# ilyakurdyukov/jpeg-quantsmooth

Measured on AMD Instinct MI355X. Metric: 8x8 blocks/s at q=3 niter=3, higher is better.
Workload: dtype f32

## Files before the change

### jpeg-quantsmooth_amd/csrc/qs_kernels.hip

```cpp
#include <hip/hip_runtime.h>
#include <stdint.h>
#include <stdlib.h>
#include "qs_device.h"
#include "qs_devfn.h"



__device__ __forceinline__ void wave_lds_sync() {
  __builtin_amdgcn_fence(__ATOMIC_RELEASE, "wavefront");
  __builtin_amdgcn_wave_barrier();
  __builtin_amdgcn_fence(__ATOMIC_ACQUIRE, "wavefront");
}

__device__ __forceinline__ uint32_t mulc(uint32_t a, int c) {
  return (uint32_t)__mul24((int)a, c);
}

__device__ __forceinline__ uint32_t lshl13_add(uint32_t x, uint32_t b) {
  uint32_t r;
  asm("v_lshl_add_u32 %0, %1, 13, %2" : "=v"(r) : "v"(x), "v"(b));
  return r;
}

__device__ __forceinline__ void idct8(uint32_t (&v)[8], uint32_t bias) {
  uint32_t z1, z2, z3, z4, z5, t0, t1, t2, t3, e0, e1, e2, e3;
  z2 = v[2]; z3 = v[6];
  z1 = mulc(z2 + z3, 4433);
  asm volatile("" : "+v"(z1));
  t2 = z1 - mulc(z3, 15137);
  t3 = z1 + mulc(z2, 6270);
  t0 = lshl13_add(v[0] + v[4], bias);
  t1 = lshl13_add(v[0] - v[4], bias);
  e0 = t0 + t3; e3 = t0 - t3; e1 = t1 + t2; e2 = t1 - t2;
  t0 = v[7]; t1 = v[5]; t2 = v[3]; t3 = v[1];
  z1 = t0 + t3; z2 = t1 + t2; z3 = t0 + t2; z4 = t1 + t3;
  z5 = mulc(z3 + z4, 9633);
  asm volatile("" : "+v"(z5));
  t0 = mulc(t0, 2446);  t1 = mulc(t1, 16819);
  t2 = mulc(t2, 25172); t3 = mulc(t3, 12299);
  z1 = mulc(z1, 7373);  z2 = mulc(z2, 20995);
  z3 = mulc(z3, 16069); z4 = mulc(z4, 3196);
  z3 = z5 - z3; z4 = z5 - z4;
  t0 += z3 - z1; t1 += z4 - z2; t2 += z3 - z2; t3 += z4 - z1;
  v[0] = e0 + t3; v[7] = e0 - t3;
  v[1] = e1 + t2; v[6] = e1 - t2;
  v[2] = e2 + t1; v[5] = e2 - t1;
  v[3] = e3 + t0; v[4] = e3 - t0;
}

__device__ __forceinline__ void idct_pass1(uint32_t (&ws)[64]) {
#pragma unroll
  for (int x = 0; x < 8; ++x) {
    uint32_t col[8];
#pragma unroll
    for (int j = 0; j < 8; ++j) col[j] = ws[j * 8 + x];
    idct8(col, 1024u);
#pragma unroll
    for (int j = 0; j < 8; ++j) ws[j * 8 + x] = (uint32_t)((int32_t)col[j] >> 11);
  }
}

__device__ __forceinline__ void idct_pass2_row(uint32_t (&row)[8], int (&out)[8]) {
  idct8(row, 257u << 17);
#pragma unroll
  for (int j = 0; j < 8; ++j) {
    int z = (int32_t)row[j];
    z = min(max(z, 0), (256 << 18) - 1);
    out[j] = z >> 18;
  }
}

#define QS_PIX_BITS 0x45000000u
__device__ __forceinline__ void idct_pass2_row_f(uint32_t (&row)[8], float (&out)[8]) {
  idct8(row, 257u << 17);
#pragma unroll
  for (int j = 0; j < 8; ++j) {
    int z = (int32_t)row[j];
    z = min(max(z, 0), (256 << 18) - 1);
    out[j] = __builtin_bit_cast(float, __builtin_amdgcn_alignbit(QS_PIX_BITS >> 14, (uint32_t)z, 18));
  }
}
__device__ __forceinline__ float pix_from_byte(uint32_t v, int n) {
  return __builtin_bit_cast(float, QS_PIX_BITS | ((v >> (8 * n)) & 0xffu));
}

__device__ __forceinline__ void
store_pixel_row(uint8_t* __restrict__ org, int pitch, int y, const int (&o)[8], int bx, int by, int wblk, int hblk,
                int rep_top, int rep_bot) {
  uint2 pk;
  pk.x = (uint32_t)o[0] | ((uint32_t)o[1] << 8) | ((uint32_t)o[2] << 16) | ((uint32_t)o[3] << 24);
  pk.y = (uint32_t)o[4] | ((uint32_t)o[5] << 8) | ((uint32_t)o[6] << 16) | ((uint32_t)o[7] << 24);
  uint8_t* rp = org + (size_t)y * pitch;
  *reinterpret_cast<uint2*>(rp) = pk;
  const bool top = (y == 0 && by == 0 && rep_top), bot = (y == 7 && by == hblk - 1 && rep_bot);
  if (bx == 0) {
    rp[-1] = (uint8_t)o[0];
    if (top) rp[-1 - pitch] = (uint8_t)o[0];
    if (bot) rp[-1 + pitch] = (uint8_t)o[0];
  }
  if (bx == wblk - 1) {
    rp[8] = (uint8_t)o[7];
    if (top) rp[8 - pitch] = (uint8_t)o[7];
    if (bot) rp[8 + pitch] = (uint8_t)o[7];
  }
  if (top) *reinterpret_cast<uint2*>(rp - pitch) = pk;
  if (bot) *reinterpret_cast<uint2*>(rp + pitch) = pk;
}

__device__ __forceinline__ void
idct_ws_to_plane(uint32_t (&ws)[64], uint8_t* __restrict__ plane, int wblk, int hblk, int pitch,
                 int rep_top, int rep_bot, int blk) {
  const int by = blk / wblk, bx = blk - by * wblk;
  idct_pass1(ws);
  uint8_t* org = plane + (size_t)(by * 8 + 1) * pitch + QS_APRON_X + bx * 8;
#pragma unroll
  for (int y = 0; y < 8; ++y) {
    uint32_t row[8]; int o[8];
#pragma unroll
    for (int j = 0; j < 8; ++j) row[j] = ws[y * 8 + j];
    idct_pass2_row(row, o);
    store_pixel_row(org, pitch, y, o, bx, by, wblk, hblk, rep_top, rep_bot);
  }
}

__device__ __forceinline__ void
idct_wave_to_plane(const QsConsts* __restrict__ cst, int16_t* __restrict__ coef,
                   uint8_t* __restrict__ plane, int wblk, int hblk, int pitch,
                   int first, int defer, int rep_top, int rep_bot, int* __restrict__ status, int base, uint32_t* lds) {
  const int lane = threadIdx.x & 63;
  const int nblk = wblk * hblk;
  const int nvec = min(64, nblk - base) * 8;
  uint4* gsrc = reinterpret_cast<uint4*>(coef) + (size_t)base * 8;
  uint4 v[8];
#pragma unroll
  for (int j = 0; j < 8; ++j) {
    const int idx = j * 64 + lane;
    v[j] = make_uint4(0, 0, 0, 0);
    if (idx < nvec) v[j] = gsrc[idx];
  }
  if (first) {
    int q[8], bad = 0;
    qs_load_qraw8(cst, lane & 7, q);
#pragma unroll
    for (int j = 0; j < 8; ++j) v[j] = qs_dequant8<true>(v[j], q, bad);
    if (!defer) {
#pragma unroll
      for (int j = 0; j < 8; ++j) {
        const int idx = j * 64 + lane;
        if (idx < nvec) gsrc[idx] = v[j];
      }
    }
    if (bad) atomicOr(status, 1);
  }
  {
    const int m0 = (lane & 7) * 4;
#pragma unroll
    for (int j = 0; j < 8; ++j) {
      uint32_t* dst = lds + m0 * QS_LDS_PITCH + (j * 8 + (lane >> 3));
      dst[0] = v[j].x; dst[QS_LDS_PITCH] = v[j].y; dst[2 * QS_LDS_PITCH] = v[j].z; dst[3 * QS_LDS_PITCH] = v[j].w;
    }
  }
  wave_lds_sync();
  const uint32_t* col = lds + lane;
  uint32_t ws[64];
#pragma unroll
  for (int r = 0; r < 32; ++r) {
    const uint32_t d = col[r * QS_LDS_PITCH];
    ws[r * 2] = (uint32_t)(int32_t)(int16_t)(d & 0xffff);
    ws[r * 2 + 1] = (uint32_t)((int32_t)d >> 16);
  }
  if (base + lane < nblk) idct_ws_to_plane(ws, plane, wblk, hblk, pitch, rep_top, rep_bot, base + lane);
}

__global__ void __launch_bounds__(256)
qs_idct_plane_kernel(const QsConsts* __restrict__ cst, int16_t* __restrict__ coef,
                     uint8_t* __restrict__ plane, int wblk, int hblk, int pitch,
                     int first, int rep_top, int rep_bot, int* __restrict__ status) {
  __shared__ uint32_t lds_all[4][32 * QS_LDS_PITCH];
  const int wave = threadIdx.x >> 6;
  const int base = __builtin_amdgcn_readfirstlane((int)(blockIdx.x * 256 + wave * 64));
  if (base >= wblk * hblk) return;
  idct_wave_to_plane(cst, coef, plane, wblk, hblk, pitch, first & 1, first & 2, rep_top, rep_bot, status, base, lds_all[wave]);
}

__global__ void __launch_bounds__(256)
qs_idct_set_kernel(const QsPlaneSet set, int first) {
  __shared__ uint32_t lds_all[4][32 * QS_LDS_PITCH];
  const int wave = threadIdx.x >> 6;
  const int w = __builtin_amdgcn_readfirstlane((int)(blockIdx.x * 4 + wave));
  if (w >= set.wave0[set.n]) return;
  const int i = qs_set_find(set, w);
  const QsPlaneRef& r = set.ref[i];
  const int base = (w - set.wave0[i]) * 64;
  if (base >= r.wblk * r.hblk) return;
  idct_wave_to_plane(r.cst, r.coef, r.plane, r.wblk, r.hblk, r.pitch, first, r.mode & QS_PLANE_QUANT,
                     r.mode & QS_PLANE_REP_TOP, r.mode & QS_PLANE_REP_BOT, r.status, base, lds_all[wave]);
}



typedef int16_t __attribute__((may_alias)) lds_i16;
__device__ __forceinline__ int lds_coef(const uint32_t* col, int i) {
  const lds_i16* p = reinterpret_cast<const lds_i16*>(col + (i >> 1) * QS_LDS_PITCH) + (i & 1);
  return *p;
}
__device__ __forceinline__ void lds_set_coef(uint32_t* col, int i, int v) {
  lds_i16* p = reinterpret_cast<lds_i16*>(col + (i >> 1) * QS_LDS_PITCH) + (i & 1);
  *p = (lds_i16)v;
}

static_assert(QS_LDS_PITCH * 4 == 260, "the literal offsets below assume a 260-byte row pitch");
#define QS_LDS16_GROUP(BASE, W, N0) \
  asm volatile("ds_read_i16 %0, %16\n\tds_read_i16 %1, %16 offset:2\n\t" \
               "ds_read_i16 %2, %16 offset:260\n\tds_read_i16 %3, %16 offset:262\n\t" \
               "ds_read_i16 %4, %16 offset:520\n\tds_read_i16 %5, %16 offset:522\n\t" \
               "ds_read_i16 %6, %16 offset:780\n\tds_read_i16 %7, %16 offset:782\n\t" \
               "ds_read_i16 %8, %16 offset:1040\n\tds_read_i16 %9, %16 offset:1042\n\t" \
               "ds_read_i16 %10, %16 offset:1300\n\tds_read_i16 %11, %16 offset:1302\n\t" \
               "ds_read_i16 %12, %16 offset:1560\n\tds_read_i16 %13, %16 offset:1562\n\t" \
               "ds_read_i16 %14, %16 offset:1820\n\tds_read_i16 %15, %16 offset:1822\n\t" \
               "s_waitcnt lgkmcnt(0)" \
               : "=&v"(W[(N0) + 0]), "=&v"(W[(N0) + 1]), "=&v"(W[(N0) + 2]), "=&v"(W[(N0) + 3]), \
                 "=&v"(W[(N0) + 4]), "=&v"(W[(N0) + 5]), "=&v"(W[(N0) + 6]), "=&v"(W[(N0) + 7]), \
                 "=&v"(W[(N0) + 8]), "=&v"(W[(N0) + 9]), "=&v"(W[(N0) + 10]), "=&v"(W[(N0) + 11]), \
                 "=&v"(W[(N0) + 12]), "=&v"(W[(N0) + 13]), "=&v"(W[(N0) + 14]), "=&v"(W[(N0) + 15]) \
               : "v"(BASE) : "memory")
__device__ __forceinline__ void lds_read_block_i16(const uint32_t* col, uint32_t (&ws)[64]) {
  typedef const __attribute__((address_space(3))) uint32_t* lds_ptr;
  const uint32_t a0 = (uint32_t)(uintptr_t)(lds_ptr)col;
  const uint32_t a1 = a0 + 8 * 260, a2 = a0 + 16 * 260, a3 = a0 + 24 * 260;
  QS_LDS16_GROUP(a0, ws, 0);
  QS_LDS16_GROUP(a1, ws, 16);
  QS_LDS16_GROUP(a2, ws, 32);
  QS_LDS16_GROUP(a3, ws, 48);
}

#define QS_PIX_SCALE 0.000244140625f
#define QS_TERM_D(D, W) { \
    float u_ = __builtin_amdgcn_fmed3f(Rs - __builtin_fabsf(D), 0.0f, 1.0f); \
    float t_ = u_ * u_; \
    float x_ = (D) * t_; \
    float y_ = (W) * t_; \
    num = num + x_ * y_; \
    den = den + y_ * y_; }
#define QS_TERM(A, B, W) { float d_ = (A) - (B); QS_TERM_D(d_, W) }

typedef float qs_w16 __attribute__((ext_vector_type(16)));
typedef int qs_i4 __attribute__((ext_vector_type(4)));
#define QS_SWAIT(BUF) asm volatile("s_waitcnt lgkmcnt(0)" : "+s"(BUF) : : "memory")

#define QS_WAVES_PER_WG 4
#define QS_SMOOTH_MIN_WAVES 3
#define QS_RESIDENT_WG (256 * QS_SMOOTH_MIN_WAVES * 4 / QS_WAVES_PER_WG)
#define QS_PRIO_SLOW 3
#define QS_PRIO_TERMS 0

#define QS_TERM_OPT(COND, A, B, W) { float d_, t_; \
        asm volatile( \
          "s_cmp_lg_u32 %[c], 0\n\t" \
          "s_cbranch_scc1 1f\n\t" \
          "v_sub_f32 %[d], %[a], %[b]\n\t" \
          "v_sub_f32 %[t], %[r], |%[d]| clamp\n\t" \
          "v_mul_f32 %[t], %[t], %[t]\n\t" \
          "v_mul_f32 %[d], %[d], %[t]\n\t" \
          "v_mul_f32 %[t], %[w], %[t]\n\t" \
          "v_mul_f32 %[d], %[d], %[t]\n\t" \
          "v_add_f32 %[n], %[n], %[d]\n\t" \
          "v_mul_f32 %[d], %[t], %[t]\n\t" \
          "v_add_f32 %[e], %[e], %[d]\n" \
          "1:" \
          : [n] "+v"(num), [e] "+v"(den), [d] "=&v"(d_), [t] "=&v"(t_) \
          : [a] "v"(A), [b] "v"(B), [w] "s"(W), [r] "s"(Rs), [c] "s"(COND) : "scc"); }
#define QS_TERM_ASM(A, B, W) { float d_, t_; \
        asm volatile( \
          "v_sub_f32 %[d], %[a], %[b]\n\t" \
          "v_sub_f32 %[t], %[r], |%[d]| clamp\n\t" \
          "v_mul_f32 %[t], %[t], %[t]\n\t" \
          "v_mul_f32 %[d], %[d], %[t]\n\t" \
          "v_mul_f32 %[t], %[w], %[t]\n\t" \
          "v_mul_f32 %[d], %[d], %[t]\n\t" \
          "v_add_f32 %[n], %[n], %[d]\n\t" \
          "v_mul_f32 %[d], %[t], %[t]\n\t" \
          "v_add_f32 %[e], %[e], %[d]" \
          : [n] "+v"(num), [e] "+v"(den), [d] "=&v"(d_), [t] "=&v"(t_) \
          : [a] "v"(A), [b] "v"(B), [w] "s"(W), [r] "s"(Rs)); }

#define QS_TERM_D_ASM(D, W) { float d_, t_; \
        asm volatile( \
          "v_sub_f32 %[t], %[r], |%[a]| clamp\n\t" \
          "v_mul_f32 %[t], %[t], %[t]\n\t" \
          "v_mul_f32 %[d], %[a], %[t]\n\t" \
          "v_mul_f32 %[t], %[w], %[t]\n\t" \
          "v_mul_f32 %[d], %[d], %[t]\n\t" \
          "v_add_f32 %[n], %[n], %[d]\n\t" \
          "v_mul_f32 %[d], %[t], %[t]\n\t" \
          "v_add_f32 %[e], %[e], %[d]" \
          : [n] "+v"(num), [e] "+v"(den), [d] "=&v"(d_), [t] "=&v"(t_) \
          : [a] "v"(D), [w] "s"(W), [r] "s"(Rs)); }
#define QS_HOIST 20
#ifndef QS_HOIST_DIAG
#define QS_HOIST_DIAG 32
#endif
#ifndef QS_Q1_SKIP
#define QS_Q1_SKIP 1
#endif
#ifndef QS_STASH
#define QS_STASH 1
#endif

#define QS_SMOOTH_KERNEL_NAME qs_smooth_plane_kernel
#include "qs_smooth_kernel.inc"
#undef QS_SMOOTH_KERNEL_NAME
#define QS_SMOOTH_KERNEL_NAME qs_smooth_set_kernel
#define QS_SMOOTH_SET 1
#include "qs_smooth_kernel.inc"
#undef QS_SMOOTH_KERNEL_NAME
#undef QS_SMOOTH_SET

#define QS_DP_KERNEL_NAME qs_smooth_dp_kernel
#include "qs_smooth_dp_kernel.inc"
#undef QS_DP_KERNEL_NAME
#define QS_DP_KERNEL_NAME qs_smooth_dp_set_kernel
#define QS_DP_SET 1
#include "qs_smooth_dp_kernel.inc"
#undef QS_DP_KERNEL_NAME
#undef QS_DP_SET

__global__ void __launch_bounds__(256)
qs_clamp_kernel(int16_t* __restrict__ coef, size_t nvec) {
  size_t i = (size_t)blockIdx.x * 256 + threadIdx.x;
  const size_t stride = (size_t)gridDim.x * 256;
  uint4* p = reinterpret_cast<uint4*>(coef);
  for (; i < nvec; i += stride) {
    uint4 v = p[i];
    uint32_t d[4] = {v.x, v.y, v.z, v.w};
#pragma unroll
    for (int c = 0; c < 4; ++c) {
      int lo = (int16_t)(d[c] & 0xffff), hi = (int32_t)d[c] >> 16;
      lo = min(max(lo, -1023), 1023); hi = min(max(hi, -1023), 1023);
      d[c] = ((uint32_t)lo & 0xffffu) | ((uint32_t)hi << 16);
    }
    p[i] = make_uint4(d[0], d[1], d[2], d[3]);
  }
}

__global__ void __launch_bounds__(256)
qs_dequant_kernel(const QsConsts* __restrict__ cst, int16_t* __restrict__ coef, size_t nvec) {
  size_t i = (size_t)blockIdx.x * 256 + threadIdx.x;
  const size_t stride = (size_t)gridDim.x * 256;
  uint4* p = reinterpret_cast<uint4*>(coef);
  for (; i < nvec; i += stride) {
    uint4 v = p[i];
    uint32_t d[4] = {v.x, v.y, v.z, v.w};
    const int j = (int)(i & 7);
#pragma unroll
    for (int c = 0; c < 4; ++c) {
      int lo = (int16_t)(d[c] & 0xffff), hi = (int32_t)d[c] >> 16;
      lo *= cst->qraw[j * 8 + c * 2]; hi *= cst->qraw[j * 8 + c * 2 + 1];
      d[c] = ((uint32_t)lo & 0xffffu) | ((uint32_t)hi << 16);
    }
    p[i] = make_uint4(d[0], d[1], d[2], d[3]);
  }
}

#include "qs_launch.h"

void qs_launch_idct_plane(const QsConsts* cst, int16_t* coef, uint8_t* plane, int wblk, int hblk,
                          int first, int rep_top, int rep_bot, int* status, hipStream_t s) {
  const int nblk = wblk * hblk;
  const int f = first == 3 ? 3 : first ? 1 : 0;
  hipLaunchKernelGGL(qs_idct_plane_kernel, dim3((nblk + 255) / 256), dim3(256), 0, s,
                     cst, coef, plane, wblk, hblk, qs_plane_pitch(wblk), f, rep_top, rep_bot, status);
}

#define QS_DP_WAVES 4
static int qs_dp_waves(int groups) {
  static const int on = [] { const char* v = getenv("QS_HIP_DP"); return v ? atoi(v) : 1; }();
  static const int lim = [] { const char* v = getenv("QS_HIP_DP_GROUPS"); return v ? atoi(v) : 768; }();
  static const int lim2 = [] { const char* v = getenv("QS_HIP_DP_GROUPS2"); return v ? atoi(v) : 1536; }();
  if (!on) return 0;
  return groups <= lim ? QS_DP_WAVES : groups <= lim2 ? 2 : 0;
}

void qs_launch_smooth_plane(const QsConsts* cst, int16_t* coef, const uint8_t* plane, uint8_t* plane_next, int rep_top, int rep_bot,
                            int wblk, int hblk, int diag, int rebalance, int final_clamp, int blk_begin, int blk_end, hipStream_t s) {
  const int n = blk_end - blk_begin;
  if (n <= 0) return;
  const int pitch = qs_plane_pitch(wblk);
  const int rep = (rep_top ? QS_PLANE_REP_TOP : 0) | (rep_bot ? QS_PLANE_REP_BOT : 0);
  if (const int nw = qs_dp_waves((n + 63) / 64)) {
    const dim3 g((n + 63) / 64), b(64 * nw);
#define QS_GO_DP(D, W) hipLaunchKernelGGL((qs_smooth_dp_kernel<D, W>), g, b, 0, s, cst, coef, plane, plane_next, rep, wblk, hblk, pitch, rebalance, final_clamp, blk_begin, blk_end)
    if (nw == 2) { if (diag) QS_GO_DP(true, 2); else QS_GO_DP(false, 2); }
    else if (diag) QS_GO_DP(true, QS_DP_WAVES); else QS_GO_DP(false, QS_DP_WAVES);
#undef QS_GO_DP
    return;
  }
  const int per_wg = 64 * QS_WAVES_PER_WG;
  const dim3 grid((n + per_wg - 1) / per_wg), block(per_wg);
#define QS_GO(K) hipLaunchKernelGGL(K, grid, block, 0, s, cst, coef, plane, plane_next, rep, wblk, hblk, pitch, rebalance, final_clamp, blk_begin, blk_end)
  if (diag) QS_GO(qs_smooth_plane_kernel<true>); else QS_GO(qs_smooth_plane_kernel<false>);
#undef QS_GO
}

void qs_launch_idct_set(const QsPlaneSet& set, int first, hipStream_t s) {
  const int nw = set.wave0[set.n];
  if (nw <= 0) return;
  hipLaunchKernelGGL(qs_idct_set_kernel, dim3((nw + 3) / 4), dim3(256), 0, s, set, first);
}

void qs_launch_smooth_set(const QsPlaneSet& set, int diag, int final_clamp, hipStream_t s) {
  const int nw = set.wave0[set.n];
  if (nw <= 0) return;
  if (const int dw = qs_dp_waves(nw)) {
    const dim3 g(nw), b(64 * dw);
#define QS_GO_DP(D, W) hipLaunchKernelGGL((qs_smooth_dp_set_kernel<D, W>), g, b, 0, s, set, final_clamp)
    if (dw == 2) { if (diag) QS_GO_DP(true, 2); else QS_GO_DP(false, 2); }
    else if (diag) QS_GO_DP(true, QS_DP_WAVES); else QS_GO_DP(false, QS_DP_WAVES);
#undef QS_GO_DP
    return;
  }
  const dim3 grid((nw + QS_WAVES_PER_WG - 1) / QS_WAVES_PER_WG), block(64 * QS_WAVES_PER_WG);
  if (diag) hipLaunchKernelGGL(qs_smooth_set_kernel<true>, grid, block, 0, s, set, final_clamp);
  else      hipLaunchKernelGGL(qs_smooth_set_kernel<false>, grid, block, 0, s, set, final_clamp);
}

void qs_launch_clamp(int16_t* coef, size_t nblk, hipStream_t s) {
  const size_t nvec = nblk * 8;
  const int grid = (int)((nvec + 255) / 256 < 8192 ? (nvec + 255) / 256 : 8192);
  hipLaunchKernelGGL(qs_clamp_kernel, dim3(grid ? grid : 1), dim3(256), 0, s, coef, nvec);
}

void qs_launch_dequant(const QsConsts* cst, int16_t* coef, size_t nblk, hipStream_t s) {
  const size_t nvec = nblk * 8;
  const int grid = (int)((nvec + 255) / 256 < 8192 ? (nvec + 255) / 256 : 8192);
  hipLaunchKernelGGL(qs_dequant_kernel, dim3(grid ? grid : 1), dim3(256), 0, s, cst, coef, nvec);
}
```

### jpeg-quantsmooth_amd/csrc/qs_smooth_kernel.inc

```
template <bool DIAG>
__global__ void __launch_bounds__(64 * QS_WAVES_PER_WG, QS_SMOOTH_MIN_WAVES)
#ifdef QS_SMOOTH_SET
QS_SMOOTH_KERNEL_NAME(const QsPlaneSet set, int final_clamp) {
  __shared__ uint32_t lds_all[QS_WAVES_PER_WG][32 * QS_LDS_PITCH];
#if QS_STASH
  __shared__ uint32_t stash_all[QS_WAVES_PER_WG][2 * 8 * 64];
#endif
  const int lane = threadIdx.x & 63, wave = threadIdx.x >> 6;
  uint32_t* lds = lds_all[wave];
  uint32_t* col = lds + lane;
  const int gw = __builtin_amdgcn_readfirstlane((int)(blockIdx.x * QS_WAVES_PER_WG + wave));
  if (gw >= set.wave0[set.n]) return;
  const int pi = qs_set_find(set, gw);
  const QsConsts* __restrict__ cst = set.ref[pi].cst;
  int16_t* __restrict__ coef = set.ref[pi].coef;
  const uint8_t* __restrict__ plane = set.ref[pi].plane;
  const int wblk = set.ref[pi].wblk, hblk = set.ref[pi].hblk, pitch = set.ref[pi].pitch;
  const int rebalance = set.ref[pi].mode & QS_PLANE_REBALANCE;
  const int nblk = wblk * hblk;
  const int base = (gw - set.wave0[pi]) * 64;
  (void)hblk;
#else
QS_SMOOTH_KERNEL_NAME(const QsConsts* __restrict__ cst, int16_t* __restrict__ coef,
                       const uint8_t* __restrict__ plane, uint8_t* __restrict__ plane_next, int rep,
                       int wblk, int hblk, int pitch,
                       int rebalance, int final_clamp, int blk_begin, int blk_end) {
  __shared__ uint32_t lds_all[QS_WAVES_PER_WG][32 * QS_LDS_PITCH];
#if QS_STASH
  __shared__ uint32_t stash_all[QS_WAVES_PER_WG][2 * 8 * 64];
#endif
  const int lane = threadIdx.x & 63, wave = threadIdx.x >> 6;
  uint32_t* lds = lds_all[wave];
  uint32_t* col = lds + lane;
  const int nblk = blk_end;
  const int base = blk_begin + (blockIdx.x * QS_WAVES_PER_WG + wave) * 64;
#endif
  if (base >= nblk) return;
  const int tail_prio = __builtin_amdgcn_readfirstlane(
      (gridDim.x > QS_RESIDENT_WG && blockIdx.x >= (gridDim.x / QS_RESIDENT_WG) * QS_RESIDENT_WG) ? 1 : 0);
  const int nvec = min(64, nblk - base) * 8;
#ifdef QS_STAGGER
  { unsigned hwid; asm volatile("s_getreg_b32 %0, hwreg(HW_REG_HW_ID)" : "=s"(hwid)); if (hwid & 1u) __builtin_amdgcn_s_sleep(QS_STAGGER); }
#endif

  uint4* gsrc = reinterpret_cast<uint4*>(coef) + (size_t)base * 8;
#ifdef QS_SMOOTH_SET
  if (set.ref[pi].mode & QS_PLANE_QUANT) {
    const int m0 = (lane & 7) * 4;
    int q[8], unused = 0;
    qs_load_qraw8(cst, lane & 7, q);
#pragma unroll
    for (int j = 0; j < 8; ++j) {
      const int idx = j * 64 + lane;
      uint4 v = make_uint4(0, 0, 0, 0);
      if (idx < nvec) v = gsrc[idx];
      v = qs_dequant8<false>(v, q, unused);
      uint32_t* dst = lds + m0 * QS_LDS_PITCH + (j * 8 + (lane >> 3));
      dst[0] = v.x; dst[QS_LDS_PITCH] = v.y; dst[2 * QS_LDS_PITCH] = v.z; dst[3 * QS_LDS_PITCH] = v.w;
    }
  } else
#endif
  {
    const int m0 = (lane & 7) * 4;
#pragma unroll
    for (int j = 0; j < 8; ++j) {
      const int idx = j * 64 + lane;
      uint4 v = make_uint4(0, 0, 0, 0);
      if (idx < nvec) v = gsrc[idx];
      uint32_t* dst = lds + m0 * QS_LDS_PITCH + (j * 8 + (lane >> 3));
      dst[0] = v.x; dst[QS_LDS_PITCH] = v.y; dst[2 * QS_LDS_PITCH] = v.z; dst[3 * QS_LDS_PITCH] = v.w;
    }
  }

  const int blk = min(base + lane, nblk - 1);
  const int by = blk / wblk, bx = blk - by * wblk;
  const uint8_t* org = plane + (size_t)(by * 8 + 1) * pitch + QS_APRON_X + bx * 8;
  uint32_t edge[8];
  {
    const uint2 t = *reinterpret_cast<const uint2*>(org - pitch);
    const uint2 b = *reinterpret_cast<const uint2*>(org + (size_t)8 * pitch);
    edge[0] = t.x; edge[1] = t.y; edge[2] = b.x; edge[3] = b.y;
    uint32_t l[8], r[8];
#pragma unroll
    for (int y = 0; y < 8; ++y) {
      l[y] = org[(ptrdiff_t)y * pitch - 1];
      r[y] = org[(ptrdiff_t)y * pitch + 8];
    }
    edge[4] = l[0] | (l[1] << 8) | (l[2] << 16) | (l[3] << 24);
    edge[5] = l[4] | (l[5] << 8) | (l[6] << 16) | (l[7] << 24);
    edge[6] = r[0] | (r[1] << 8) | (r[2] << 16) | (r[3] << 24);
    edge[7] = r[4] | (r[5] << 8) | (r[6] << 16) | (r[7] << 24);
  }
  wave_lds_sync();

  constexpr int TS = DIAG ? 272 : 160;
  float px[64];
  float bd[32];
  constexpr int NH = DIAG ? QS_HOIST_DIAG : QS_HOIST;
  float hd[NH];

  int kfirst = 63;
#if QS_STASH
  int stash_hi = 0;
#endif
  uint32_t chg = 0;
  long long reb_m0 = 0, reb_m1 = 0;
  const float* tabp = cst->tab;
  const int32_t* recp = &cst->rec[0][0];
  qs_w16 WA, WB;
  qs_i4 REC;
  qs_i4 RECN;
  asm volatile("s_load_dwordx4 %0, %2, %3\n\ts_load_dwordx16 %1, %4, %5\n\ts_waitcnt lgkmcnt(0)"
               : "=&s"(REC), "=&s"(WA) : "s"(recp), "s"(63u * 16u), "s"(tabp), "s"((uint32_t)63 * (TS * 4)) : "memory");
  RECN = REC;

#pragma unroll 1
  for (int g = 0; g < 14; ++g) {
    __builtin_amdgcn_s_setprio(QS_PRIO_SLOW);
    if (g == 0 || __builtin_amdgcn_ballot_w64(chg != 0) != 0) {
      chg = 0;
      uint32_t ws[64];
      lds_read_block_i16(col, ws);
#if QS_STASH
      {
        uint32_t* stash = stash_all[wave] + lane;
#pragma unroll
        for (int x = 0; x < 8; ++x) {
          uint32_t c[8];
          const bool low = x <= 1, high = x >= 6;
          const int slot = (x == 0 || x == 7) ? 0 : 1;
          bool reuse = false, store = false;
          if (low) { reuse = g >= 1 && g <= 7 - x; store = g == 0; }
          if (high) {
            const int fin = 15 - x;
            const bool have = (stash_hi >> (x - 6)) & 1;
            reuse = g >= fin && have; store = g >= fin && !have;
          }
          if ((low || high) && reuse) {
#pragma unroll
            for (int j = 0; j < 8; ++j) c[j] = stash[(slot * 8 + j) * 64];
          } else {
#pragma unroll
            for (int j = 0; j < 8; ++j) c[j] = ws[j * 8 + x];
            idct8(c, 1024u);
#pragma unroll
            for (int j = 0; j < 8; ++j) c[j] = (uint32_t)((int32_t)c[j] >> 11);
            if ((low || high) && store) {
#pragma unroll
              for (int j = 0; j < 8; ++j) stash[(slot * 8 + j) * 64] = c[j];
              if (high) stash_hi |= 1 << (x - 6);
            }
          }
#pragma unroll
          for (int j = 0; j < 8; ++j) ws[j * 8 + x] = c[j];
        }
      }
#else
      idct_pass1(ws);
#endif
#pragma unroll
      for (int y = 0; y < 8; ++y) {
        uint32_t row[8]; float o[8];
#pragma unroll
        for (int j = 0; j < 8; ++j) row[j] = ws[y * 8 + j];
        idct_pass2_row_f(row, o);
#pragma unroll
        for (int j = 0; j < 8; ++j) px[y * 8 + j] = o[j];
      }
#pragma unroll
      for (int e = 0; e < 8; ++e) asm volatile("" : "+v"(edge[e]));
#pragma unroll
      for (int x = 0; x < 8; ++x) {
        bd[x]      = px[x]         - pix_from_byte(edge[0 + (x >> 2)], x & 3);
        bd[8 + x]  = px[56 + x]    - pix_from_byte(edge[2 + (x >> 2)], x & 3);
        bd[16 + x] = px[x * 8]     - pix_from_byte(edge[4 + (x >> 2)], x & 3);
        bd[24 + x] = px[x * 8 + 7] - pix_from_byte(edge[6 + (x >> 2)], x & 3);
      }
#pragma unroll
      for (int t = 0; t < NH; ++t) hd[t] = px[(t / 7) * 8 + t % 7] - px[(t / 7) * 8 + t % 7 + 1];
    }
    const int len = min(g + 1, 15 - g);
    const int klast = max(kfirst - len + 1, 1);
#pragma unroll 1
    for (int k = kfirst; k >= klast; --k) {
#pragma unroll
      for (int p = 0; p < 64; ++p) asm volatile("" : "+v"(px[p]));
      const int md = REC[3];
      const int x2k = (REC[0] >> 16) & 31, qk = REC[1] & 0xffff, x1k = REC[1] >> 16;
      const uint32_t lds_off = ((uint32_t)md >> QS_REC_LDS_SHIFT) & 0x3fffu;
      int rs_bits = REC[2];
      asm volatile("" : "+s"(rs_bits));
      const float Rs = __builtin_bit_cast(float, rs_bits);
      const uint32_t kb = (uint32_t)k * (TS * 4);
      const uint32_t kb_nxt = kb - (uint32_t)(TS * 4);
      const uint32_t kb_s = (uint32_t)__builtin_amdgcn_readfirstlane((int)kb);
      const uint32_t kb_nxt_s = (uint32_t)__builtin_amdgcn_readfirstlane((int)kb_nxt);
      const uint32_t next_first = kb_nxt + (((uint32_t)md >> QS_REC_NXT_SHIFT) & 0x100u);
      const uint32_t after_V = DIAG ? kb + 640u : next_first;
      const uint32_t after_B = (md & QS_REC_V_ANY) ? kb + 384u : after_V;
#if QS_Q1_SKIP
      if (__builtin_expect(md & QS_REC_Q1, 0)) {
        {
          const int c0 = *reinterpret_cast<lds_i16*>(reinterpret_cast<char*>(col) + lds_off);
          reb_m0 += (long long)(c0 * c0);
          reb_m1 += (long long)(c0 * c0);
        }
        asm volatile("s_load_dwordx16 %0, %2, %3\n\ts_load_dwordx4 %1, %4, %5\n\ts_waitcnt lgkmcnt(0)"
                     : "=&s"(WA), "=&s"(RECN)
                     : "s"(tabp), "s"((uint32_t)__builtin_amdgcn_readfirstlane((int)next_first)), "s"(recp),
                       "s"((uint32_t)(k - 1) * 16u) : "memory");
        REC = RECN;
      } else
#endif
      {
      float num = 0.0f, den = 0.0f;
      asm volatile("s_setprio %c1\n\ts_cmp_eq_u32 %0, 0\n\ts_cbranch_scc1 1f\n\ts_setprio %c2\n1:"
                   : : "s"(tail_prio), "i"(QS_PRIO_TERMS), "i"(QS_PRIO_TERMS + 1) : "scc");

#define QS_ROW_D(W, Y) { \
        _Pragma("unroll") for (int x = 0; x < 7; ++x) { \
          QS_TERM(px[(Y) * 8 + x], px[(Y) * 8 + x + 9], W[x]) \
          QS_TERM(px[(Y) * 8 + x + 1], px[(Y) * 8 + x + 8], W[8 + x]) } }
#define QS_EDGE16(W, J0) { \
        _Pragma("unroll") for (int j = 0; j < 16; ++j) QS_TERM_D(bd[(J0) + j], W[j]) }
#define QS_HOISTED_TERM(T, WT) else if ((T) < NH) QS_TERM_D_ASM(hd[(T) % NH], WT)
#define QS_ROWS_H_M(W, Y0, MODE) { \
        _Pragma("unroll") for (int yy = 0; yy < 2; ++yy) \
        _Pragma("unroll") for (int x = 0; x < 7; ++x) { \
          if (((MODE) == 2 && (x & 1)) || ((MODE) == 1 && x == 3)) {} \
          QS_HOISTED_TERM(((Y0) + yy) * 7 + x, W[yy * 8 + x]) \
          else QS_TERM_ASM(px[((Y0) + yy) * 8 + x], px[((Y0) + yy) * 8 + x + 1], W[yy * 8 + x]) } }
#define QS_ROWS_V_M(W, Y0, NY, MODE) { \
        _Pragma("unroll") for (int yy = 0; yy < (NY); ++yy) \
        _Pragma("unroll") for (int x = 0; x < 8; ++x) { \
          if (((MODE) == 2 && (((Y0) + yy) & 1)) || ((MODE) == 1 && (Y0) + yy == 3)) {} \
          else QS_TERM_ASM(px[((Y0) + yy) * 8 + x], px[((Y0) + yy) * 8 + x + 8], W[yy * 8 + x]) } }

      const uint32_t rec_next = (uint32_t)(k - 1) * 16u;
#define QS_ISSUE(NXT, BYTEOFF) \
      asm volatile("s_load_dwordx16 %0, %3, %4" : "=&s"(NXT), "+v"(num), "+v"(den) \
                   : "s"(tabp), "s"((uint32_t)__builtin_amdgcn_readfirstlane((int)(BYTEOFF))) : "memory")
#define QS_ISSUE_K(NXT, IMM) \
      asm volatile("s_load_dwordx16 %0, %3, %4 offset:%c5" : "=&s"(NXT), "+v"(num), "+v"(den) \
                   : "s"(tabp), "s"(kb_s), "i"(IMM) : "memory")
#define QS_LAND(NXT) asm volatile("s_waitcnt lgkmcnt(0)" : "+s"(NXT), "+v"(num), "+v"(den) : : "memory")
#define QS_ISSUE_R(NXT, BYTEOFF) \
      asm volatile("s_load_dwordx16 %0, %4, %5\n\ts_load_dwordx4 %1, %6, %7" : "=&s"(NXT), "=&s"(RECN), "+v"(num), "+v"(den) \
                   : "s"(tabp), "s"((uint32_t)__builtin_amdgcn_readfirstlane((int)(BYTEOFF))), "s"(recp), "s"(rec_next) : "memory")
#define QS_LAND_R(NXT) asm volatile("s_waitcnt lgkmcnt(0)" : "+s"(NXT), "+s"(RECN), "+v"(num), "+v"(den) : : "memory")
#define QS_T4(O) "s_load_dword %1, %4, %5 offset:" #O "\n\ts_load_dword %1, %4, %5 offset:" #O "+0x40\n\ts_load_dword %1, %4, %5 offset:" #O "+0x80\n\ts_load_dword %1, %4, %5 offset:" #O "+0xc0\n\t"
#define QS_ISSUE_T(NXT, IMM) \
      uint32_t touch; \
      if (DIAG) asm volatile("s_load_dwordx16 %0, %4, %6 offset:%c7\n\t" QS_T4(0x0) QS_T4(0x100) QS_T4(0x200) QS_T4(0x300) "s_load_dword %1, %4, %5 offset:0x400" \
                   : "=&s"(NXT), "=&s"(touch), "+v"(num), "+v"(den) \
                   : "s"(tabp), "s"(kb_nxt_s), "s"(kb_s), "i"(IMM) : "memory"); \
      else      asm volatile("s_load_dwordx16 %0, %4, %6 offset:%c7\n\t" QS_T4(0x0) QS_T4(0x100) "s_load_dword %1, %4, %5 offset:0x200\n\ts_load_dword %1, %4, %5 offset:0x240" \
                   : "=&s"(NXT), "=&s"(touch), "+v"(num), "+v"(den) \
                   : "s"(tabp), "s"(kb_nxt_s), "s"(kb_s), "i"(IMM) : "memory")
#define QS_LAND_T(NXT) asm volatile("s_waitcnt lgkmcnt(0)" : "+s"(NXT), "+s"(touch), "+v"(num), "+v"(den) : : "memory")
#define QS_H_SECTION(MODE) { \
        QS_ISSUE_K(WB, 64);  QS_ROWS_H_M(WA, 0, MODE) QS_LAND(WB); \
        QS_ISSUE_K(WA, 128); QS_ROWS_H_M(WB, 2, MODE) QS_LAND(WA); \
        QS_ISSUE_K(WB, 192); QS_ROWS_H_M(WA, 4, MODE) QS_LAND(WB); \
        QS_ISSUE_K(WA, 256); QS_ROWS_H_M(WB, 6, MODE) QS_LAND(WA); }
      if (md & QS_REC_H_ANY) {
        if (md & QS_REC_H_SKIP4) QS_H_SECTION(2)
        else if (md & QS_REC_H_EVEN) QS_H_SECTION(1)
        else QS_H_SECTION(0)
      }
      QS_ISSUE_T(WB, 320); QS_EDGE16(WA, 0) QS_LAND_T(WB);
      if (!DIAG && !(md & QS_REC_V_ANY)) { QS_ISSUE_R(WA, after_B); QS_EDGE16(WB, 16) QS_LAND_R(WA); }
      else                   { QS_ISSUE(WA, after_B);   QS_EDGE16(WB, 16) QS_LAND(WA); }
#define QS_V_SECTION(MODE) { \
        QS_ISSUE_K(WB, 448); QS_ROWS_V_M(WA, 0, 2, MODE) QS_LAND(WB); \
        QS_ISSUE_K(WA, 512); QS_ROWS_V_M(WB, 2, 2, MODE) QS_LAND(WA); \
        QS_ISSUE_K(WB, 576); QS_ROWS_V_M(WA, 4, 2, MODE) QS_LAND(WB); \
        if (!DIAG) { QS_ISSUE_R(WA, after_V); QS_ROWS_V_M(WB, 6, 1, MODE) QS_LAND_R(WA); } \
        else       { QS_ISSUE(WA, after_V);   QS_ROWS_V_M(WB, 6, 1, MODE) QS_LAND(WA); } }
      if (md & QS_REC_V_ANY) {
        if (md & QS_REC_V_SKIP4) QS_V_SECTION(2)
        else if (md & QS_REC_V_EVEN) QS_V_SECTION(1)
        else QS_V_SECTION(0)
      }
      if (DIAG) {
        QS_ISSUE_K(WB, 704);  QS_ROW_D(WA, 0) QS_LAND(WB);
        QS_ISSUE_K(WA, 768);  QS_ROW_D(WB, 1) QS_LAND(WA);
        QS_ISSUE_K(WB, 832);  QS_ROW_D(WA, 2) QS_LAND(WB);
        QS_ISSUE_K(WA, 896);  QS_ROW_D(WB, 3) QS_LAND(WA);
        QS_ISSUE_K(WB, 960);  QS_ROW_D(WA, 4) QS_LAND(WB);
        QS_ISSUE_K(WA, 1024); QS_ROW_D(WB, 5) QS_LAND(WA);
        QS_ISSUE_R(WB, next_first); QS_ROW_D(WA, 6) QS_LAND_R(WB);
        WA = WB;
      }
#undef QS_ROWS_H_M
#undef QS_HOISTED_TERM
#undef QS_ROWS_V_M
#undef QS_H_SECTION
#undef QS_V_SECTION
#undef QS_ISSUE
#undef QS_ISSUE_K
#undef QS_LAND
#undef QS_ISSUE_R
#undef QS_LAND_R
#undef QS_ISSUE_T
#undef QS_LAND_T
#undef QS_T4

      __builtin_amdgcn_s_setprio(QS_PRIO_SLOW);
      lds_i16* const cptr = reinterpret_cast<lds_i16*>(reinterpret_cast<char*>(col) + lds_off);
      const int c0 = *cptr;
      const int r = f2i_x86(round_half_away((num / den) * 4096.0f));
      {
        int orig, lo, hi;
        interval(c0, qk, x1k, x2k, orig, lo, hi);
        int v = (int)((uint32_t)c0 - (uint32_t)r);
        v = min(max(v, lo), hi);
        *cptr = (lds_i16)v;
        chg |= (uint32_t)(v ^ c0);
        if (rebalance) {
          reb_m0 += (long long)(v * orig);
          reb_m1 += (long long)(orig * orig);
        }
      }
      REC = RECN;
      }
    }
    kfirst = klast - 1;
  }
  QS_SWAIT(WA);

  if (rebalance) {
    const long long m0 = reb_m0, m1 = reb_m1;
    if (m1 > m0) {
      const int mul = (int)(((m1 << 13) + (m0 >> 1)) / m0);
#pragma unroll 9
      for (int n = 1; n < 64; ++n) {
        const int c = lds_coef(col, n);
        int orig, lo, hi;
        interval(c, cst->qn[n], cst->x1n[n], cst->x2n[n], orig, lo, hi);
        int v = (c * mul + 0x1000) >> 13;
        v = min(max(v, lo), hi);
        lds_set_coef(col, n, v);
      }
    }
  }
  wave_lds_sync();

  {
    int lane2 = lane;
    asm volatile("" : "+v"(lane2));
    const int lane = lane2;
    const int m0 = (lane & 7) * 4;
#pragma unroll
    for (int j = 0; j < 8; ++j) {
      const int idx = j * 64 + lane;
      const uint32_t* s = lds + m0 * QS_LDS_PITCH + (j * 8 + (lane >> 3));
      uint32_t d[4] = {s[0], s[QS_LDS_PITCH], s[2 * QS_LDS_PITCH], s[3 * QS_LDS_PITCH]};
      if (final_clamp) {
#pragma unroll
        for (int c = 0; c < 4; ++c) {
          int lo = (int16_t)(d[c] & 0xffff), hi = (int32_t)d[c] >> 16;
          lo = min(max(lo, -1023), 1023); hi = min(max(hi, -1023), 1023);
          d[c] = ((uint32_t)lo & 0xffffu) | ((uint32_t)hi << 16);
        }
      }
      if (idx < nvec) gsrc[idx] = make_uint4(d[0], d[1], d[2], d[3]);
    }
  }

#ifdef QS_SMOOTH_SET
  int pi2 = pi;
  asm volatile("" : "+s"(pi2));
  uint8_t* __restrict__ plane_next = set.ref[pi2].plane_next;
  const int rep = set.ref[pi2].mode, wblk2 = set.ref[pi2].wblk, hblk2 = set.ref[pi2].hblk, pitch2 = set.ref[pi2].pitch;
#else
  const int wblk2 = wblk, hblk2 = hblk, pitch2 = pitch;
#endif
  if (plane_next) {
    uint32_t ws[64];
    lds_read_block_i16(col, ws);
    if (base + lane < nblk)
      idct_ws_to_plane(ws, plane_next, wblk2, hblk2, pitch2, rep & QS_PLANE_REP_TOP, rep & QS_PLANE_REP_BOT, base + lane);
  }
}

#undef QS_ROW_D
#undef QS_EDGE16
```

Measured before the change: 276.3 million.

## Precompute pixel differences and move per-lane state to LDS in non-diagonal smoothing

For the non-diagonal kernel variant, the 64-entry pixel array is replaced with precomputed horizontal and vertical difference arrays. The edge bytes, stash and rebalance accumulators move into a per-wave LDS extension, with the accumulators updated through wave-scope LDS atomics, and the change test becomes a wave ballot. The aim is to cut VGPR use and per-term subtraction work so the kernel fits three waves per SIMD. A slow path recomputes the rebalance sums and widens the intervals when large coefficients could overflow, and a Python script is added to check the VGPR, scratch and LDS budget. The extra LDS per wave and the atomic traffic could reduce occupancy or add latency.

```diff
diff --git a/jpeg-quantsmooth_amd/csrc/check_kernel_budget.py b/jpeg-quantsmooth_amd/csrc/check_kernel_budget.py
--- /dev/null
+++ b/jpeg-quantsmooth_amd/csrc/check_kernel_budget.py
@@ -0,0 +1,49 @@
+#!/usr/bin/env python3
+import re
+import sys
+
+KERNELS = ("qs_smooth_plane_kernel", "qs_smooth_set_kernel")
+MAX_VGPRS = 168
+MAX_LDS = 160 * 1024 // 3
+FIELDS = ("group_segment_fixed_size", "private_segment_fixed_size", "vgpr_count")
+
+
+def kernel_records(text):
+    m = re.search(r"^\s*\.amdgpu_metadata\s*$(.*?)^\s*\.end_amdgpu_metadata\s*$", text, re.S | re.M)
+    if not m:
+        return {}
+    recs, cur = [], None
+    for line in m.group(1).split("\n"):
+        if re.match(r"  - \.", line):
+            cur = {}
+            recs.append(cur)
+            line = "    " + line[4:]
+        f = re.match(r"    \.(\w+):\s*(\S+)\s*$", line)
+        if f and cur is not None:
+            cur[f.group(1)] = f.group(2)
+    return {r["name"]: {k: int(r[k]) for k in FIELDS if k in r} for r in recs if "name" in r}
+
+
+def main(path):
+    recs = {n: r for n, r in kernel_records(open(path).read()).items() if any(k in n for k in KERNELS)}
+    if len(recs) != 4 or any(len(r) != len(FIELDS) for r in recs.values()):
+        print(f"check_kernel_budget: ERROR: expected the metadata of 4 recovery kernels in {path}, found {sorted(recs)}", file=sys.stderr)
+        return 1
+    bad = 0
+    for n, r in sorted(recs.items()):
+        why = []
+        if r["private_segment_fixed_size"] != 0:
+            why.append(f"{r['private_segment_fixed_size']} B of scratch per lane (spills)")
+        if r["vgpr_count"] > MAX_VGPRS:
+            why.append(f"{r['vgpr_count']} VGPRs > {MAX_VGPRS} (three waves per SIMD)")
+        if r["group_segment_fixed_size"] > MAX_LDS:
+            why.append(f"{r['group_segment_fixed_size']} B of LDS > {MAX_LDS} (three workgroups per CU)")
+        print(f"check_kernel_budget: {n}: {r['vgpr_count']} VGPRs, {r['private_segment_fixed_size']} B scratch, "
+              f"{r['group_segment_fixed_size']} B LDS" + (" -- ERROR: " + "; ".join(why) if why else ""),
+              file=sys.stderr if why else sys.stdout)
+        bad += bool(why)
+    return 1 if bad else 0
+
+
+if __name__ == "__main__":
+    sys.exit(main(sys.argv[1]))
diff --git a/jpeg-quantsmooth_amd/csrc/qs_kernels.hip b/jpeg-quantsmooth_amd/csrc/qs_kernels.hip
--- a/jpeg-quantsmooth_amd/csrc/qs_kernels.hip
+++ b/jpeg-quantsmooth_amd/csrc/qs_kernels.hip
@@ -210,15 +210,15 @@
 }
 
 static_assert(QS_LDS_PITCH * 4 == 260, "the literal offsets below assume a 260-byte row pitch");
-#define QS_LDS16_GROUP(BASE, W, N0) \
-  asm volatile("ds_read_i16 %0, %16\n\tds_read_i16 %1, %16 offset:2\n\t" \
-               "ds_read_i16 %2, %16 offset:260\n\tds_read_i16 %3, %16 offset:262\n\t" \
-               "ds_read_i16 %4, %16 offset:520\n\tds_read_i16 %5, %16 offset:522\n\t" \
-               "ds_read_i16 %6, %16 offset:780\n\tds_read_i16 %7, %16 offset:782\n\t" \
-               "ds_read_i16 %8, %16 offset:1040\n\tds_read_i16 %9, %16 offset:1042\n\t" \
-               "ds_read_i16 %10, %16 offset:1300\n\tds_read_i16 %11, %16 offset:1302\n\t" \
-               "ds_read_i16 %12, %16 offset:1560\n\tds_read_i16 %13, %16 offset:1562\n\t" \
-               "ds_read_i16 %14, %16 offset:1820\n\tds_read_i16 %15, %16 offset:1822\n\t" \
+#define QS_LDS16_GROUP(BASE, W, N0, O) \
+  asm volatile("ds_read_i16 %0, %16 offset:" #O "\n\tds_read_i16 %1, %16 offset:" #O "+2\n\t" \
+               "ds_read_i16 %2, %16 offset:" #O "+260\n\tds_read_i16 %3, %16 offset:" #O "+262\n\t" \
+               "ds_read_i16 %4, %16 offset:" #O "+520\n\tds_read_i16 %5, %16 offset:" #O "+522\n\t" \
+               "ds_read_i16 %6, %16 offset:" #O "+780\n\tds_read_i16 %7, %16 offset:" #O "+782\n\t" \
+               "ds_read_i16 %8, %16 offset:" #O "+1040\n\tds_read_i16 %9, %16 offset:" #O "+1042\n\t" \
+               "ds_read_i16 %10, %16 offset:" #O "+1300\n\tds_read_i16 %11, %16 offset:" #O "+1302\n\t" \
+               "ds_read_i16 %12, %16 offset:" #O "+1560\n\tds_read_i16 %13, %16 offset:" #O "+1562\n\t" \
+               "ds_read_i16 %14, %16 offset:" #O "+1820\n\tds_read_i16 %15, %16 offset:" #O "+1822\n\t" \
                "s_waitcnt lgkmcnt(0)" \
                : "=&v"(W[(N0) + 0]), "=&v"(W[(N0) + 1]), "=&v"(W[(N0) + 2]), "=&v"(W[(N0) + 3]), \
                  "=&v"(W[(N0) + 4]), "=&v"(W[(N0) + 5]), "=&v"(W[(N0) + 6]), "=&v"(W[(N0) + 7]), \
@@ -229,10 +229,18 @@
   typedef const __attribute__((address_space(3))) uint32_t* lds_ptr;
   const uint32_t a0 = (uint32_t)(uintptr_t)(lds_ptr)col;
   const uint32_t a1 = a0 + 8 * 260, a2 = a0 + 16 * 260, a3 = a0 + 24 * 260;
-  QS_LDS16_GROUP(a0, ws, 0);
-  QS_LDS16_GROUP(a1, ws, 16);
-  QS_LDS16_GROUP(a2, ws, 32);
-  QS_LDS16_GROUP(a3, ws, 48);
+  QS_LDS16_GROUP(a0, ws, 0, 0);
+  QS_LDS16_GROUP(a1, ws, 16, 0);
+  QS_LDS16_GROUP(a2, ws, 32, 0);
+  QS_LDS16_GROUP(a3, ws, 48, 0);
+}
+__device__ __forceinline__ void lds_read_block_i16_1(const uint32_t* col, uint32_t (&ws)[64]) {
+  typedef const __attribute__((address_space(3))) uint32_t* lds_ptr;
+  const uint32_t a0 = (uint32_t)(uintptr_t)(lds_ptr)col;
+  QS_LDS16_GROUP(a0, ws, 0, 0);
+  QS_LDS16_GROUP(a0, ws, 16, 2080);
+  QS_LDS16_GROUP(a0, ws, 32, 4160);
+  QS_LDS16_GROUP(a0, ws, 48, 6240);
 }
 
 #define QS_PIX_SCALE 0.000244140625f
@@ -297,7 +305,6 @@
           "v_add_f32 %[e], %[e], %[d]" \
           : [n] "+v"(num), [e] "+v"(den), [d] "=&v"(d_), [t] "=&v"(t_) \
           : [a] "v"(D), [w] "s"(W), [r] "s"(Rs)); }
-#define QS_HOIST 20
 #ifndef QS_HOIST_DIAG
 #define QS_HOIST_DIAG 32
 #endif
@@ -307,6 +314,22 @@
 #ifndef QS_STASH
 #define QS_STASH 1
 #endif
+#define QS_X_STASH 0
+#define QS_X_EDGE 8
+#define QS_X_REB 16
+#define QS_X_DWORDS 20
+static_assert(QS_WAVES_PER_WG * (32 * QS_LDS_PITCH + QS_X_DWORDS * 64) * 4 <= 160 * 1024 / 3, "LDS budget of three workgroups per CU");
+typedef unsigned long long __attribute__((address_space(3))) qs_lds_u64;
+__device__ __forceinline__ void qs_lds_add64(qs_lds_u64* p, long long v) {
+  __hip_atomic_fetch_add(p, (unsigned long long)v, __ATOMIC_RELAXED, __HIP_MEMORY_SCOPE_WAVEFRONT);
+}
+__device__ __forceinline__ qs_lds_u64* qs_xreb(const uint32_t* col, const uint32_t* lds, int n) {
+  typedef const __attribute__((address_space(3))) uint32_t* lds_ptr;
+  uint32_t a = (uint32_t)(uintptr_t)(lds_ptr)col;
+  asm volatile("" : "+v"(a));
+  const uint32_t b = (uint32_t)(uintptr_t)(lds_ptr)lds;
+  return (qs_lds_u64*)(a * 2u - b + (uint32_t)((32 * QS_LDS_PITCH + (QS_X_REB + 2 * n) * 64) * 4));
+}
 
 #define QS_SMOOTH_KERNEL_NAME qs_smooth_plane_kernel
 #include "qs_smooth_kernel.inc"
diff --git a/jpeg-quantsmooth_amd/csrc/qs_smooth_kernel.inc b/jpeg-quantsmooth_amd/csrc/qs_smooth_kernel.inc
--- a/jpeg-quantsmooth_amd/csrc/qs_smooth_kernel.inc
+++ b/jpeg-quantsmooth_amd/csrc/qs_smooth_kernel.inc
@@ -2,11 +2,11 @@
 __global__ void __launch_bounds__(64 * QS_WAVES_PER_WG, QS_SMOOTH_MIN_WAVES)
 #ifdef QS_SMOOTH_SET
 QS_SMOOTH_KERNEL_NAME(const QsPlaneSet set, int final_clamp) {
-  __shared__ uint32_t lds_all[QS_WAVES_PER_WG][32 * QS_LDS_PITCH];
+  __shared__ __attribute__((aligned(16))) uint32_t lds_all[QS_WAVES_PER_WG][32 * QS_LDS_PITCH + (DIAG ? 0 : QS_X_DWORDS * 64)];
 #if QS_STASH
   __shared__ uint32_t stash_all[QS_WAVES_PER_WG][2 * 8 * 64];
 #endif
-  const int lane = threadIdx.x & 63, wave = threadIdx.x >> 6;
+  const int lane = threadIdx.x & 63, wave = DIAG ? (int)(threadIdx.x >> 6) : __builtin_amdgcn_readfirstlane((int)(threadIdx.x >> 6));
   uint32_t* lds = lds_all[wave];
   uint32_t* col = lds + lane;
   const int gw = __builtin_amdgcn_readfirstlane((int)(blockIdx.x * QS_WAVES_PER_WG + wave));
@@ -25,11 +25,11 @@
                        const uint8_t* __restrict__ plane, uint8_t* __restrict__ plane_next, int rep,
                        int wblk, int hblk, int pitch,
                        int rebalance, int final_clamp, int blk_begin, int blk_end) {
-  __shared__ uint32_t lds_all[QS_WAVES_PER_WG][32 * QS_LDS_PITCH];
+  __shared__ __attribute__((aligned(16))) uint32_t lds_all[QS_WAVES_PER_WG][32 * QS_LDS_PITCH + (DIAG ? 0 : QS_X_DWORDS * 64)];
 #if QS_STASH
   __shared__ uint32_t stash_all[QS_WAVES_PER_WG][2 * 8 * 64];
 #endif
-  const int lane = threadIdx.x & 63, wave = threadIdx.x >> 6;
+  const int lane = threadIdx.x & 63, wave = DIAG ? (int)(threadIdx.x >> 6) : __builtin_amdgcn_readfirstlane((int)(threadIdx.x >> 6));
   uint32_t* lds = lds_all[wave];
   uint32_t* col = lds + lane;
   const int nblk = blk_end;
@@ -44,6 +44,8 @@
 #endif
 
   uint4* gsrc = reinterpret_cast<uint4*>(coef) + (size_t)base * 8;
+  uint32_t bigacc = 0;
+#define QS_BIG_ACC(V) if constexpr (!DIAG) bigacc |= ((V).x ^ ((V).x << 1)) | ((V).y ^ ((V).y << 1)) | ((V).z ^ ((V).z << 1)) | ((V).w ^ ((V).w << 1))
 #ifdef QS_SMOOTH_SET
   if (set.ref[pi].mode & QS_PLANE_QUANT) {
     const int m0 = (lane & 7) * 4;
@@ -55,6 +57,7 @@
       uint4 v = make_uint4(0, 0, 0, 0);
       if (idx < nvec) v = gsrc[idx];
       v = qs_dequant8<false>(v, q, unused);
+      QS_BIG_ACC(v);
       uint32_t* dst = lds + m0 * QS_LDS_PITCH + (j * 8 + (lane >> 3));
       dst[0] = v.x; dst[QS_LDS_PITCH] = v.y; dst[2 * QS_LDS_PITCH] = v.z; dst[3 * QS_LDS_PITCH] = v.w;
     }
@@ -67,6 +70,7 @@
       const int idx = j * 64 + lane;
       uint4 v = make_uint4(0, 0, 0, 0);
       if (idx < nvec) v = gsrc[idx];
+      QS_BIG_ACC(v);
       uint32_t* dst = lds + m0 * QS_LDS_PITCH + (j * 8 + (lane >> 3));
       dst[0] = v.x; dst[QS_LDS_PITCH] = v.y; dst[2 * QS_LDS_PITCH] = v.z; dst[3 * QS_LDS_PITCH] = v.w;
     }
@@ -91,19 +95,29 @@
     edge[6] = r[0] | (r[1] << 8) | (r[2] << 16) | (r[3] << 24);
     edge[7] = r[4] | (r[5] << 8) | (r[6] << 16) | (r[7] << 24);
   }
+  uint32_t* const xcol = col + 32 * QS_LDS_PITCH;
+  if constexpr (!DIAG) {
+#pragma unroll
+    for (int e = 0; e < 8; ++e) xcol[(QS_X_EDGE + e) * 64] = edge[e];
+    *qs_xreb(col, lds, 0) = 0; *qs_xreb(col, lds, 1) = 0;
+  }
   wave_lds_sync();
 
   constexpr int TS = DIAG ? 272 : 160;
-  float px[64];
+  float px[DIAG ? 64 : 1];
   float bd[32];
-  constexpr int NH = DIAG ? QS_HOIST_DIAG : QS_HOIST;
+  constexpr int NH = DIAG ? QS_HOIST_DIAG : 1;
   float hd[NH];
+  float dh[DIAG ? 1 : 56], dv[DIAG ? 1 : 56];
 
   int kfirst = 63;
 #if QS_STASH
   int stash_hi = 0;
 #endif
   uint32_t chg = 0;
+  uint64_t chg_any = 0;
+#undef QS_BIG_ACC
+  const bool big_wave = !DIAG && __builtin_amdgcn_ballot_w64((bigacc & 0xC000C000u) != 0) != 0;
   long long reb_m0 = 0, reb_m1 = 0;
   const float* tabp = cst->tab;
   const int32_t* recp = &cst->rec[0][0];
@@ -117,17 +131,18 @@
 #pragma unroll 1
   for (int g = 0; g < 14; ++g) {
     __builtin_amdgcn_s_setprio(QS_PRIO_SLOW);
-    if (g == 0 || __builtin_amdgcn_ballot_w64(chg != 0) != 0) {
+    if (g == 0 || (DIAG ? __builtin_amdgcn_ballot_w64(chg != 0) != 0 : chg_any != 0)) {
       chg = 0;
+      chg_any = 0;
       uint32_t ws[64];
-      lds_read_block_i16(col, ws);
+      if constexpr (DIAG) lds_read_block_i16(col, ws); else lds_read_block_i16_1(col, ws);
 #if QS_STASH
       {
-        uint32_t* stash = stash_all[wave] + lane;
+        uint32_t* stash = DIAG ? stash_all[wave] + lane : xcol + QS_X_STASH * 64;
 #pragma unroll
         for (int x = 0; x < 8; ++x) {
           uint32_t c[8];
-          const bool low = x <= 1, high = x >= 6;
+          const bool low = x <= (DIAG ? 1 : 0), high = x >= (DIAG ? 6 : 7);
           const int slot = (x == 0 || x == 7) ? 0 : 1;
           bool reuse = false, store = false;
           if (low) { reuse = g >= 1 && g <= 7 - x; store = g == 0; }
@@ -158,6 +173,35 @@
 #else
       idct_pass1(ws);
 #endif
+      if constexpr (!DIAG) {
+        float prev[8];
+#pragma unroll
+        for (int y = 0; y < 8; ++y) {
+          uint32_t row[8]; float o[8];
+#pragma unroll
+          for (int j = 0; j < 8; ++j) row[j] = ws[y * 8 + j];
+          idct_pass2_row_f(row, o);
+#pragma unroll
+          for (int x = 0; x < 7; ++x) dh[y * 7 + x] = o[x] - o[x + 1];
+          if (y > 0) {
+#pragma unroll
+            for (int x = 0; x < 8; ++x) dv[(y - 1) * 8 + x] = prev[x] - o[x];
+          }
+          if (y == 0 || y == 7) {
+            const uint32_t e0 = xcol[(QS_X_EDGE + (y ? 2 : 0)) * 64], e1 = xcol[(QS_X_EDGE + (y ? 3 : 1)) * 64];
+#pragma unroll
+            for (int x = 0; x < 8; ++x) bd[(y ? 8 : 0) + x] = o[x] - pix_from_byte(x < 4 ? e0 : e1, x & 3);
+          }
+          {
+            const uint32_t el = xcol[(QS_X_EDGE + 4 + (y >> 2)) * 64], er = xcol[(QS_X_EDGE + 6 + (y >> 2)) * 64];
+            bd[16 + y] = o[0] - pix_from_byte(el, y & 3);
+            bd[24 + y] = o[7] - pix_from_byte(er, y & 3);
+          }
+#pragma unroll
+          for (int x = 0; x < 8; ++x) prev[x] = o[x];
+          __builtin_amdgcn_sched_barrier(0);
+        }
+      } else {
 #pragma unroll
       for (int y = 0; y < 8; ++y) {
         uint32_t row[8]; float o[8];
@@ -178,13 +222,16 @@
       }
 #pragma unroll
       for (int t = 0; t < NH; ++t) hd[t] = px[(t / 7) * 8 + t % 7] - px[(t / 7) * 8 + t % 7 + 1];
+      }
     }
     const int len = min(g + 1, 15 - g);
     const int klast = max(kfirst - len + 1, 1);
 #pragma unroll 1
     for (int k = kfirst; k >= klast; --k) {
-#pragma unroll
-      for (int p = 0; p < 64; ++p) asm volatile("" : "+v"(px[p]));
+      if constexpr (DIAG) {
+#pragma unroll
+        for (int p = 0; p < 64; ++p) asm volatile("" : "+v"(px[p]));
+      }
       const int md = REC[3];
       const int x2k = (REC[0] >> 16) & 31, qk = REC[1] & 0xffff, x1k = REC[1] >> 16;
       const uint32_t lds_off = ((uint32_t)md >> QS_REC_LDS_SHIFT) & 0x3fffu;
@@ -202,8 +249,14 @@
       if (__builtin_expect(md & QS_REC_Q1, 0)) {
         {
           const int c0 = *reinterpret_cast<lds_i16*>(reinterpret_cast<char*>(col) + lds_off);
-          reb_m0 += (long long)(c0 * c0);
-          reb_m1 += (long long)(c0 * c0);
+          if constexpr (DIAG) {
+            reb_m0 += (long long)(c0 * c0);
+            reb_m1 += (long long)(c0 * c0);
+          } else {
+            qs_lds_u64* const xreb = qs_xreb(col, lds, 0);
+            qs_lds_add64(xreb, (long long)(c0 * c0));
+            qs_lds_add64(xreb + 64, (long long)(c0 * c0));
+          }
         }
         asm volatile("s_load_dwordx16 %0, %2, %3\n\ts_load_dwordx4 %1, %4, %5\n\ts_waitcnt lgkmcnt(0)"
                      : "=&s"(WA), "=&s"(RECN)
@@ -222,18 +275,22 @@
           QS_TERM(px[(Y) * 8 + x], px[(Y) * 8 + x + 9], W[x]) \
           QS_TERM(px[(Y) * 8 + x + 1], px[(Y) * 8 + x + 8], W[8 + x]) } }
 #define QS_EDGE16(W, J0) { \
-        _Pragma("unroll") for (int j = 0; j < 16; ++j) QS_TERM_D(bd[(J0) + j], W[j]) }
+        _Pragma("unroll") for (int j = 0; j < 16; ++j) { \
+          if constexpr (DIAG) QS_TERM_D(bd[(J0) + j], W[j]) \
+          else QS_TERM_D_ASM(bd[(J0) + j], W[j]) } }
 #define QS_HOISTED_TERM(T, WT) else if ((T) < NH) QS_TERM_D_ASM(hd[(T) % NH], WT)
 #define QS_ROWS_H_M(W, Y0, MODE) { \
         _Pragma("unroll") for (int yy = 0; yy < 2; ++yy) \
         _Pragma("unroll") for (int x = 0; x < 7; ++x) { \
           if (((MODE) == 2 && (x & 1)) || ((MODE) == 1 && x == 3)) {} \
+          else if constexpr (!DIAG) QS_TERM_D_ASM(dh[((Y0) + yy) * 7 + x], W[yy * 8 + x]) \
           QS_HOISTED_TERM(((Y0) + yy) * 7 + x, W[yy * 8 + x]) \
           else QS_TERM_ASM(px[((Y0) + yy) * 8 + x], px[((Y0) + yy) * 8 + x + 1], W[yy * 8 + x]) } }
 #define QS_ROWS_V_M(W, Y0, NY, MODE) { \
         _Pragma("unroll") for (int yy = 0; yy < (NY); ++yy) \
         _Pragma("unroll") for (int x = 0; x < 8; ++x) { \
           if (((MODE) == 2 && (((Y0) + yy) & 1)) || ((MODE) == 1 && (Y0) + yy == 3)) {} \
+          else if constexpr (!DIAG) QS_TERM_D_ASM(dv[((Y0) + yy) * 8 + x], W[yy * 8 + x]) \
           else QS_TERM_ASM(px[((Y0) + yy) * 8 + x], px[((Y0) + yy) * 8 + x + 8], W[yy * 8 + x]) } }
 
       const uint32_t rec_next = (uint32_t)(k - 1) * 16u;
@@ -315,11 +372,22 @@
         interval(c0, qk, x1k, x2k, orig, lo, hi);
         int v = (int)((uint32_t)c0 - (uint32_t)r);
         v = min(max(v, lo), hi);
-        *cptr = (lds_i16)v;
-        chg |= (uint32_t)(v ^ c0);
-        if (rebalance) {
-          reb_m0 += (long long)(v * orig);
-          reb_m1 += (long long)(orig * orig);
+        if constexpr (DIAG) {
+          *cptr = (lds_i16)v;
+          chg |= (uint32_t)(v ^ c0);
+          if (rebalance) {
+            reb_m0 += (long long)(v * orig);
+            reb_m1 += (long long)(orig * orig);
+          }
+        } else {
+          if (__builtin_expect(big_wave, 0)) { asm volatile("" : "+v"(v)); v = r ? v : c0; }
+          *cptr = (lds_i16)v;
+          chg_any |= __builtin_amdgcn_ballot_w64(v != c0);
+          if (rebalance) {
+            qs_lds_u64* const xreb = qs_xreb(col, lds, 0);
+            qs_lds_add64(xreb, (long long)(v * orig));
+            qs_lds_add64(xreb + 64, (long long)(orig * orig));
+          }
         }
       }
       REC = RECN;
@@ -330,7 +398,19 @@
   QS_SWAIT(WA);
 
   if (rebalance) {
-    const long long m0 = reb_m0, m1 = reb_m1;
+    long long m0 = DIAG ? reb_m0 : (long long)*qs_xreb(col, lds, 0), m1 = DIAG ? reb_m1 : (long long)*qs_xreb(col, lds, 1);
+    const bool big = big_wave;
+    if (big) {
+      m0 = 0; m1 = 0;
+#pragma unroll 1
+      for (int n = 1; n < 64; ++n) {
+        const int c = lds_coef(col, n);
+        int orig, lo, hi;
+        interval(c, cst->qn[n], cst->x1n[n], cst->x2n[n], orig, lo, hi);
+        m0 += (long long)(c * orig);
+        m1 += (long long)(orig * orig);
+      }
+    }
     if (m1 > m0) {
       const int mul = (int)(((m1 << 13) + (m0 >> 1)) / m0);
 #pragma unroll 9
@@ -338,6 +418,11 @@
         const int c = lds_coef(col, n);
         int orig, lo, hi;
         interval(c, cst->qn[n], cst->x1n[n], cst->x2n[n], orig, lo, hi);
+        if (big) {
+          const int div = cst->qn[n], a = (int16_t)orig;
+          hi = a + (a < 0 ? div >> 1 : (div - 1) >> 1);
+          lo = a - (a > 0 ? div >> 1 : (div - 1) >> 1);
+        }
         int v = (c * mul + 0x1000) >> 13;
         v = min(max(v, lo), hi);
         lds_set_coef(col, n, v);
@@ -347,7 +432,7 @@
   wave_lds_sync();
 
   {
-    int lane2 = lane;
+    int lane2 = DIAG ? lane : (int)__builtin_amdgcn_mbcnt_hi(~0u, __builtin_amdgcn_mbcnt_lo(~0u, 0u));
     asm volatile("" : "+v"(lane2));
     const int lane = lane2;
     const int m0 = (lane & 7) * 4;
@@ -378,9 +463,11 @@
 #endif
   if (plane_next) {
     uint32_t ws[64];
-    lds_read_block_i16(col, ws);
-    if (base + lane < nblk)
-      idct_ws_to_plane(ws, plane_next, wblk2, hblk2, pitch2, rep & QS_PLANE_REP_TOP, rep & QS_PLANE_REP_BOT, base + lane);
+    if constexpr (DIAG) lds_read_block_i16(col, ws); else lds_read_block_i16_1(col, ws);
+    int lane3 = DIAG ? lane : (int)__builtin_amdgcn_mbcnt_hi(~0u, __builtin_amdgcn_mbcnt_lo(~0u, 0u));
+    if constexpr (!DIAG) asm volatile("" : "+v"(lane3));
+    if (base + lane3 < nblk)
+      idct_ws_to_plane(ws, plane_next, wblk2, hblk2, pitch2, rep & QS_PLANE_REP_TOP, rep & QS_PLANE_REP_BOT, base + lane3);
   }
 }
 
```

Measured after the change: 283.1 million, median of 6. 1.02x the previous value.
